# jjhbw/GoMILP

Measured on AMD Instinct MI355X. Metric: simplex pivots/sec on 2048x4096 fp64 dense LP, higher is better.
Workload: dtype f64

## Files before the change

gomilp_amd/csrc/btg_kernels.hip:

```cpp
#include <hip/hip_runtime.h>
#include <hip/hip_ext.h>
#include <stdint.h>

#include <algorithm>
#include <type_traits>

#include "device_types.h"
#include "kernels_common.h"
#include "bt_loop.h"

namespace gomilp {

namespace {

struct XWin { double m; unsigned int i; double p0, p1, p2, p3; };
struct BtWinG { double m; unsigned int i; };

}

template <int G, int NT, int RI, int KR, bool STAMP, bool LOOP = false>
__device__ __forceinline__ void bt_innerG_body(const BTArgs &a, const int g, const int nupd = 0) {
    constexpr int NW = NT / 64;
    static_assert(!LOOP || KR == 16 || KR == 24 || KR == 32, "loop mode: KR / 2 lagging + KR / 2 current terms");
    constexpr int KB = LOOP ? KR / 2 : KR;
    static_assert(G == 2 || G == 4 || G == 8 || G == 16, "G");
#ifdef GOMILP_DEBUG
    if (a.fault && g == 1) return;
#endif
    __shared__ double redM[16];
    __shared__ unsigned int redI[16];
    __shared__ double pay[16][4];
    __shared__ int s_ok;
    __shared__ unsigned long long s_acc[STAMP ? 16 : 1][16];
    unsigned long long tprev = 0;
    auto stamp = [&](int seg) {
        if constexpr (STAMP) {
            unsigned long long t;
            __builtin_amdgcn_sched_barrier(0);
            asm volatile("s_memtime %0\n\ts_waitcnt lgkmcnt(0)" : "=s"(t)::"memory");
            __builtin_amdgcn_sched_barrier(0);
            if (seg >= 0 && (threadIdx.x & 63) == 0) s_acc[threadIdx.x >> 6][seg] += t - tprev;
            tprev = t;
        }
    };
    DevState *st = a.st;
    const int tid = threadIdx.x, lane = tid & 63, wv = tid >> 6;
    const int wbase = __builtin_amdgcn_readfirstlane(tid & ~63);
    const int done = __hip_atomic_load(&st->done, __ATOMIC_RELAXED, __HIP_MEMORY_SCOPE_AGENT);
    long long xs = (long long)a.xbuf[0];
    xpair *recs = reinterpret_cast<xpair *>(a.xbuf + kXHeader);
    const double inf = __builtin_inf();
    const unsigned int ldt = (unsigned int)a.ldt;
    const char *Tb = reinterpret_cast<const char *>(a.T);
    auto ldT = [&](unsigned int elem) -> double {
        if constexpr (LOOP) return ld_agent(reinterpret_cast<const double *>(Tb + (elem << 3)));
// ... 28 lines not shown
    auto hand_on = [&](int nb) {
        hdr_out[0] = (double)(unsigned int)(blk_base + (unsigned int)G * (unsigned int)nb);
#pragma unroll
        for (int j = 0; j < 4; j++) hdr_out[1 + j] = (double)(unsigned int)(upd_base[j] + (unsigned int)nupd * (unsigned int)(nb > j ? (nb - 1 - j) / 4 + 1 : 0));
    };
    if (done) {
        if constexpr (LOOP) {
            if (tid == 0) {
                if (g == 0) {
                    __hip_atomic_store(&st->kdone2[0], 0, __ATOMIC_RELAXED, __HIP_MEMORY_SCOPE_AGENT);
                    asm volatile("s_waitcnt vmcnt(0)" ::: "memory");
                }
                __hip_atomic_fetch_add(blk_cnt, 1u, __ATOMIC_RELAXED, __HIP_MEMORY_SCOPE_AGENT);
                if (g == 0) {
                    st->tsel2[a.par ^ 1] = sel0;
                    st->loop_blocks = 0;
                    hand_on(1);
                }
            }
        } else if (g == 0 && tid == 0) st->kdone = 0;
        return;
    }
    double ureg[RI][KR], vreg[RI][KR];
#pragma unroll
    for (int s = 0; s < RI; s++) {
#pragma unroll
        for (int j = 0; j < KR; j++) { ureg[s][j] = 0; vreg[s][j] = 0; }
    }
    if constexpr (STAMP) { if (tid < 256) s_acc[tid >> 4][tid & 15] = 0; }
    __syncthreads();
    int kd = 0, status = ST_RUNNING, blands = 0;
    bool dead = false;
    long long trace_len = 0, npiv = 0;
    if (g == 0 && tid == 0) { trace_len = st->trace_len; npiv = st->pivots; }

    auto wave_first_min = [&](const double (&val)[RI]) -> BtWinG {
        double x = val[0];
#pragma unroll
        for (int s = 1; s < RI; s++) x = vmin_f64(x, val[s]);
        BtWinG w;
        w.m = wave_min_f64(x);
        w.i = 0xFFFFFFFFu;
#pragma unroll
        for (int s = RI - 1; s >= 0; s--) {
            const unsigned long long mask = __ballot(val[s] == w.m);
            if (mask) w.i = (unsigned int)((s * G + g) * NT + wbase + __builtin_ctzll(mask));
        }
        return w;
    };
    auto xchg = [&](int which) -> XWin {
        stamp(which * 5 + 0);
        if constexpr (!LOOP) asm volatile("s_waitcnt vmcnt(0)" ::: "memory");
        __syncthreads();
        stamp(which * 5 + 1);
        xs += 1;
        const double seqd = (double)xs;
        const int par = (int)(xs & 1);
        if (wv == 0) {
            double fm, v0;
            unsigned int fi;
            if constexpr (LOOP && (NW == 4 || NW == 8)) {
                const double mw = lane < NW ? redM[lane & (NW - 1)] : inf;
                const double iw = lane < NW ? (double)redI[lane & (NW - 1)] : 4294967295.0;
                double xm = mw;
                xm = vmin_f64(xm, dpp_f64<0xB1>(xm));
                xm = vmin_f64(xm, dpp_f64<0x4E>(xm));
// ... 91 lines not shown
            XLoad<1>::run(src, got, fast);
            if (__all(!act || got[0].x == seqd)) break;
            if (++spins > kXSpinLimit) { dead = true; break; }
        }
        stamp(which * 5 + 3);
        const double val = got[0].y;
        double xm = (lane < G) ? val : inf;
        xm = vmin_f64(xm, dpp_f64<0xB1>(xm));
        xm = vmin_f64(xm, dpp_f64<0x4E>(xm));
        xm = vmin_f64(xm, dpp_f64<0x141>(xm));
        const double idxl = dpp_f64<0x108>(val);
        const bool mine = lane < G && val == xm;
        double km = mine ? idxl : 4294967295.0;
        km = vmin_f64(km, dpp_f64<0xB1>(km));
        km = vmin_f64(km, dpp_f64<0x4E>(km));
        km = vmin_f64(km, dpp_f64<0x141>(km));
        const unsigned int mk = (unsigned int)(__ballot(mine && idxl == km) & 0xFFull);
        const int gw = mk ? __builtin_ctz(mk) : 0;
        const double bm = readlane_f64(xm, 0), bi = readlane_f64(km, 0);
        XWin r;
        r.m = bm;
        r.i = (unsigned int)bi;
        r.p0 = readlane_f64(val, 16 + gw);
        r.p1 = readlane_f64(val, 24 + gw);
        r.p2 = readlane_f64(val, 32 + gw);
        r.p3 = readlane_f64(val, 48 + gw);
        if (first) {
            fast = !dead && __all(!(act && (lane >> 3) == 5) || val == (double)myxcc);
            first = false;
        }
        stamp(which * 5 + 4);
        return r;
    };
    auto reduce_cols = [&](const double (&val)[RI]) -> XWin {
        const BtWinG w = wave_first_min(val);
#pragma unroll
        for (int s = 0; s < RI; s++)
            if ((unsigned int)gidx(s) == w.i) {
                pay[wv][0] = rv[s];
                pay[wv][1] = (double)nbasv[s];
                pay[wv][3] = vreg[s][0];
            }
        if (lane == 0) { redM[wv] = w.m; redI[wv] = w.i; }
        return xchg(0);
    };
    auto reduce_rows = [&](const double (&val)[RI], const double (&dcol)[RI]) -> XWin {
        const BtWinG w = wave_first_min(val);
#pragma unroll
        for (int s = 0; s < RI; s++)
            if ((unsigned int)gidx(s) == w.i) {
                pay[wv][0] = dcol[s];
                pay[wv][1] = xbv[s];
                pay[wv][2] = (double)basv[s];
                pay[wv][3] = ureg[s][0];
            }
        if (lane == 0) { redM[wv] = w.m; redI[wv] = w.i; }
        return xchg(1);
    };
    auto column = [&](int q, int k, double (&dcol)[RI], double newest) {
        double d0[RI];
#pragma unroll
        for (int s = 0; s < RI; s++) {
            const int i = gidx(s);
            const unsigned int ic = (unsigned int)(i < a.m ? i : a.m - 1);
            d0[s] = ldT(tile_off_g(ic, (unsigned int)q, ldt));
        }
        double vq[KR];
        if constexpr (LOOP) {
            const int l = lane & 31;
            const int trow = l < k ? cur0 + k - 1 - l : lag0 + nl - 1 - (l - k);
            double tv = l < k + nl ? ld_term(a.V + (size_t)trow * a.ldt + q) : 0.0;
            if (l == 0 && k + nl > 0) tv = newest;
            if constexpr (STAMP) { asm volatile("s_waitcnt vmcnt(0)" ::: "memory"); stamp(11); }
#pragma unroll
            for (int jj = 0; jj < KR; jj++) vq[jj] = readlane_f64(tv, jj);
        } else {
#pragma unroll
            for (int jj = 0; jj < KR; jj++) vq[jj] = jj < k ? ld_term(a.V + (size_t)(k - 1 - jj) * a.ldt + q) : 0.0;
        }
#pragma unroll
// ... 185 lines not shown
            if (j < a.ldt) {
                double v;
                if constexpr (LOOP) {
                    double acc[4] = {0, 0, 0, 0};
#pragma unroll
                    for (int jj = 0; jj < KR; jj++) acc[jj & 3] = __builtin_fma(up[jj], vreg[s][jj], acc[jj & 3]);
                    v = vrow[s] + ((acc[0] + acc[1]) + (acc[2] + acc[3]));
                } else {
                    v = vrow[s];
#pragma unroll
                    for (int jj = 0; jj < KR; jj++) v = __builtin_fma(up[jj], vreg[s][jj], v);
                }
                rv[s] = (j == q) ? -mult : __builtin_fma(-mult, v, rv[s]);
                const double vprime = (j == q) ? dpv + 1.0 : v;
                st_term(Vk + j, vprime);
#pragma unroll
                for (int jj = KR - 1; jj > 0; jj--) vreg[s][jj] = vreg[s][jj - 1];
                vreg[s][0] = vprime;
                if (j == q && commit_lists) nbasv[s] = lea;
            }
        }
        if constexpr (STAMP && !LOOP) asm volatile("s_waitcnt vmcnt(0)" ::: "memory");
        stamp(10);
        if (forced && a.forced_nocommit == 3) status = ST_FORCED_DONE;
        if (g == 0 && tid == 0 && !(forced && a.forced_nocommit)) {
            if (a.trace && trace_len < a.trace_cap) {
                DevPivot &tr = a.trace[trace_len];
                tr.phase = a.phase; tr.bland = bland ? 1 : 0; tr.min_idx = q; tr.replace = p; tr.entering = ent; tr.leaving = lea;
            }
            trace_len += 1;
            npiv += 1;
        }
        kd = k + 1;
    }
    nbe = blk + 1;
    if constexpr (LOOP) {
        if (dead) status = ST_XCHG_TIMEOUT;
        asm volatile("s_waitcnt vmcnt(0)" ::: "memory");
        __syncthreads();
        if (tid == 0) {
            if (g == 0) {
                __hip_atomic_store(&st->kdone2[blk & 1], kd, __ATOMIC_RELAXED, __HIP_MEMORY_SCOPE_AGENT);
                if (status != ST_RUNNING) {
                    __hip_atomic_store(&st->status, status, __ATOMIC_RELAXED, __HIP_MEMORY_SCOPE_AGENT);
                    __hip_atomic_store(&st->done, 1, __ATOMIC_RELAXED, __HIP_MEMORY_SCOPE_AGENT);
                }
                asm volatile("s_waitcnt vmcnt(0)" ::: "memory");
            }
            __hip_atomic_fetch_add(blk_cnt, 1u, __ATOMIC_RELAXED, __HIP_MEMORY_SCOPE_AGENT);
        }
        if (status != ST_RUNNING) break;
    }
    }
    if (dead) status = ST_XCHG_TIMEOUT;
    if constexpr (STAMP) {
        if (a.stamps && g == 0 && lane == 0) {
            for (int sg = 0; sg < 16; sg++) a.stamps[wv * 16 + sg] += s_acc[wv][sg];
            if (wv == 0) a.stamps[16 * 16] += (unsigned long long)kd;
        }
    }
#pragma unroll
    for (int s = 0; s < RI; s++) {
        const int i = gidx(s);
        if (i < a.ldt) a.r[i] = i < a.nn ? rv[s] : 0.0;
        if (i < a.ldu) a.xb[i] = xbv[s];
        if (i < a.m) a.basic[i] = basv[s];
        if (i < a.nn) a.nonbasic[i] = nbasv[s];
    }
    if (tid == 0 && (g == 0 || dead)) {
        if (g == 0) {
            st->trace_len = trace_len;
            st->pivots = npiv;
            if constexpr (LOOP) {
                const int napplied = kd > 0 ? nbe : nbe - 1;
                st->tsel2[a.par ^ 1] = sel0 ^ (napplied & 1);
                st->loop_blocks = nbe;
                hand_on(nbe);
            } else {
                st->kdone = kd;
            }
            st->bland_steps += blands;
            a.xbuf[0] = (double)xs;
        }
        if (status != ST_RUNNING) { st->done = 1; st->status = status; }
    }
}

template <int G, int NT, int RI, int KR, bool STAMP = false>
__global__ __launch_bounds__(NT) void k_bt_innerG(BTArgs a) {
    if (blockIdx.x & 7u) return;
    bt_innerG_body<G, NT, RI, KR, STAMP>(a, (int)(blockIdx.x >> 3));
}
template <int G, int NT, int RI, bool STAMP = false, int KB = 8>
__global__ __launch_bounds__(NT) void k_bt_loop(BTArgs a) {
    const int b = (int)blockIdx.x, x = a.xcd & 7;
    const int nupd = (a.upd_cap > 0 && a.upd_cap < (int)gridDim.x - G) ? a.upd_cap : (int)gridDim.x - G;
    if ((b & 7) == x && (b >> 3) < G) { bt_innerG_body<G, NT, RI, 2 * KB, STAMP, true>(a, b >> 3, nupd); return; }
    const int before = b <= x ? 0 : min(G, ((b - x - 1) >> 3) + 1);
    if (b - before >= nupd) return;
    bt_loop_update_role<NT, KB>(a, b - before, nupd, G);
}

template <int G, int NT, int RI, int KR>
__global__ __launch_bounds__(NT) void k_bt_innerG_batch(const BatchLP *__restrict__ lps, const int *__restrict__ ids, const int *__restrict__ count, int xcd_off) {
    const unsigned int x8 = ((blockIdx.x & 7u) + 8u - (unsigned int)xcd_off) & 7u, j = blockIdx.x >> 3;
    const int lpos = (int)((j / G) * 8u + x8);
    if (lpos >= *count) return;
    const BatchLP &lp = lps[ids[lpos]];
    const int stage = lp.stage;
    if (stage == BS_DONE || stage == BS_HOST) return;
    const BTArgs a = lp.bt;
    bt_innerG_body<G, NT, RI, KR, false>(a, (int)(j % G));
}


size_t bt_xbuf_doubles() { return (size_t)kXSync + kXSyncDoubles; }

BtGroupCfg bt_group_cfg(int m, int ldt, int knob) {
    BtGroupCfg c = {0, 0, 0};
    if (knob < 0) return c;
    const int need = m > ldt ? m : ldt;
    auto fits = [&](int G, int nt, int ri) { return (long)G * nt * ri >= need; };
    if (knob == 16) {
        if (need <= 2048) c = {8, 256, 1};
        else if (need <= 4096) c = {8, 512, 1};
        return c;
    }
    if (knob == 2 || knob == 4 || knob == 8) {
        const int G = knob;
        if (fits(G, 512, 1)) c = {G, 512, 1};
        else if (fits(G, 512, 2)) c = {G, 512, 2};
        return c;
    }
    if (knob != 0) return c;
    if (need <= 1024) return c;
    if (need <= 2048) return {8, 256, 1};
    if (need <= 4096) return {8, 512, 1};
    if (need <= 8192) return {8, 512, 2};
    return c;
}

template <int G, int NT, int RI>
static void btg_launch(const BTArgs &a, hipStream_t s, hipEvent_t e0, hipEvent_t e1) {
    if constexpr (RI == 1) {
        if (a.stamps) { hipExtLaunchKernelGGL((k_bt_innerG<G, NT, RI, 16, true>), dim3(8 * G), dim3(NT), 0, s, e0, e1, 0, a); return; }
    }
    hipExtLaunchKernelGGL((k_bt_innerG<G, NT, RI, 16>), dim3(8 * G), dim3(NT), 0, s, e0, e1, 0, a);
}
void launch_bt_inner_groups(const BTArgs &a, hipStream_t s, hipEvent_t e0, hipEvent_t e1) {
    const int G = a.groups, ri = a.group_ri;
    if (a.group_nt == 256) { btg_launch<8, 256, 1>(a, s, e0, e1); return; }
    if (G == 2) { if (ri == 1) btg_launch<2, 512, 1>(a, s, e0, e1); else btg_launch<2, 512, 2>(a, s, e0, e1); }
    else if (G == 4) { if (ri == 1) btg_launch<4, 512, 1>(a, s, e0, e1); else btg_launch<4, 512, 2>(a, s, e0, e1); }
    else { if (ri == 1) btg_launch<8, 512, 1>(a, s, e0, e1); else btg_launch<8, 512, 2>(a, s, e0, e1); }
}
bool bt_loop_supported(const BtGroupCfg &c) { return c.groups >= 2 && c.ri == 1; }
void launch_bt_loop(const BTArgs &a, int ncu, hipStream_t s, hipEvent_t e0, hipEvent_t e1) {
    const int G = a.groups;
    const unsigned int grid = (unsigned int)std::max(ncu, 8 * G);
    if (a.group_nt == 256 && G == 8) {
        if (a.stamps) hipExtLaunchKernelGGL((k_bt_loop<8, 256, 1, true>), dim3(grid), dim3(256), 0, s, e0, e1, 0, a);
        else hipExtLaunchKernelGGL((k_bt_loop<8, 256, 1>), dim3(grid), dim3(256), 0, s, e0, e1, 0, a);
        return;
    }
    if (G == 16 && a.group_nt == 128) { hipExtLaunchKernelGGL((k_bt_loop<16, 128, 1, false, 8>), dim3(std::max(grid, 136u)), dim3(128), 0, s, e0, e1, 0, a); return; }
    if (G == 16 && a.kmax == 12) { hipExtLaunchKernelGGL((k_bt_loop<16, 256, 1, false, 12>), dim3(std::max(grid, 136u)), dim3(256), 0, s, e0, e1, 0, a); return; }
    if (G == 16) { hipExtLaunchKernelGGL((k_bt_loop<16, 256, 1, false, 16>), dim3(std::max(grid, 128u)), dim3(256), 0, s, e0, e1, 0, a); return; }
    if (G == 2) hipExtLaunchKernelGGL((k_bt_loop<2, 512, 1>), dim3(grid), dim3(512), 0, s, e0, e1, 0, a);
    else if (G == 4) hipExtLaunchKernelGGL((k_bt_loop<4, 512, 1>), dim3(grid), dim3(512), 0, s, e0, e1, 0, a);
    else if (a.kmax == 16) hipExtLaunchKernelGGL((k_bt_loop<8, 512, 1, false, 16>), dim3(grid), dim3(512), 0, s, e0, e1, 0, a);
    else hipExtLaunchKernelGGL((k_bt_loop<8, 512, 1>), dim3(grid), dim3(512), 0, s, e0, e1, 0, a);
}
void launch_bt_inner_groups_batch(const BatchLP *lps, const int *ids, const int *count, int nlp, const BtGroupCfg &c, hipStream_t s, hipEvent_t e0, hipEvent_t e1, int xcd_off) {
    const unsigned int grid = 64u * (unsigned int)((nlp + 7) / 8);
    if (c.nt == 256) hipExtLaunchKernelGGL((k_bt_innerG_batch<8, 256, 1, 16>), dim3(grid), dim3(256), 0, s, e0, e1, 0, lps, ids, count, xcd_off);
    else hipExtLaunchKernelGGL((k_bt_innerG_batch<8, 512, 1, 16>), dim3(grid), dim3(512), 0, s, e0, e1, 0, lps, ids, count, xcd_off);
}
const char *bt_group_kernel_name(int G, int ri) {
    static const char *names[3][2] = {{"k_bt_innerG<2,512,1,16>", "k_bt_innerG<2,512,2,16>"}, {"k_bt_innerG<4,512,1,16>", "k_bt_innerG<4,512,2,16>"},
                                      {"k_bt_innerG<8,512,1,16>", "k_bt_innerG<8,512,2,16>"}};
    return names[G == 2 ? 0 : G == 4 ? 1 : 2][ri == 1 ? 0 : 1];
}

}
```

gomilp_amd/csrc/c_api.cpp:

```cpp
#include <math.h>
#include <stdint.h>
#include <stdio.h>
#include <stdlib.h>
#include <string.h>

#include <atomic>
#include <chrono>
#include <condition_variable>
#include <deque>
#include <functional>
#include <map>
#include <memory>
#include <mutex>
#include <string>
#include <thread>
#include <vector>

#include "engine.hpp"
#include "engine_batch.hpp"
#include "engine_batch_revised.hpp"
#include "lu_host.h"

using gomilp::BatchEngine;
using gomilp::Engine;
// ... 696 lines not shown
    return norm * gomilp::inverse_norm1_estimate(inv, (int)n, inf != 0);
}

int gomilp_debug_gonum_lu_cond(const double *M, int64_t n, int transposed, double *cond) {
    if (!M || !cond || n < 1 || n > gomilp::kGonumCondMax) return -1;
    bool dz = false;
    if (!gomilp::gonum_lu_cond(M, (int)n, (int)n, transposed != 0, cond, &dz)) return -1;
    return dz ? 1 : 0;
}

int gomilp_debug_lu_host_solve(int64_t m, int64_t nd, const int32_t *dl, const int32_t *phys, const double *diag, const double *W, int coupled,
                               const double *rhs, double *x) {
    if (m < 1 || m > 16384 || nd < 0 || nd > m || !phys || !diag || !rhs || !x || (nd > 0 && (!dl || !W))) return -1;
    const int64_t nx = coupled ? nd : m;
    for (int64_t i = 0; i < nx; i++) x[i] = 0.0;
    if (gomilp::lu_det_is_zero(diag, phys, (int)m)) return 1;
    if (coupled) {
        std::vector<double> xdl((size_t)nd);
        gomilp::lu_host_solve_coupled((int)nd, dl, phys, diag, W, rhs, xdl.data(), x);
    } else gomilp::lu_host_solve((int)m, (int)nd, dl, phys, diag, W, rhs, x);
    return 0;
}

int64_t gomilp_debug_find_independent_device(gomilp_ctx *ctx, int64_t problem, int64_t *idx_out, int64_t cap) {
    if (!ctx || !idx_out) return -GOMILP_ERR_BAD_SHAPE;
    std::vector<int32_t> idx;
    const int rc = ctx->eng->debug_find_independent(problem, idx);
    if (rc != GOMILP_OK && rc != GOMILP_ERR_SINGULAR) return -rc;
    for (size_t k = 0; k < idx.size() && (int64_t)k < cap; k++) idx_out[k] = idx[k];
    return (int64_t)idx.size();
}

long long gomilp_debug_loop_rep_launches(void) { return gomilp::bt_loop_rep_launches(); }
#ifdef GOMILP_DEBUG
void gomilp_debug_luc_stamps(unsigned long long *out) { gomilp::luc_stamps_read(out); }
void gomilp_debug_lux_stamps(unsigned long long *out) { gomilp::lux_stamps_read(out); }
void gomilp_debug_res_stamps(unsigned long long *out) { gomilp::res_stamps_read(out); }
#endif

int64_t gomilp_lp_last_trace(gomilp_ctx *ctx, gomilp_pivot *out, int64_t cap) {
    if (!ctx) return -1;
    return ctx->eng->last_trace(out, cap);
}

namespace {
constexpr int kFlatMaxCtx = 32;
struct FlatPool {
    std::mutex mu;
    std::condition_variable cv;
    std::vector<gomilp_ctx *> free_list;
    int created = 0;
};
FlatPool &flat_pool(int dev) {
    static std::mutex mu;
    static std::map<int, FlatPool *> pools;
    std::lock_guard<std::mutex> g(mu);
    auto it = pools.find(dev);
    if (it == pools.end()) it = pools.emplace(dev, new FlatPool).first;
    return *it->second;
}
}

int gomilp_lp_simplex(const double *c, const double *A, int64_t lda, const double *b, int64_t m, int64_t n, double tol,
                      const int64_t *initial_basic, double *opt_f, double *opt_x, int32_t *has_x, int64_t *basis_out,
                      gomilp_lp_stats *stats) {
    if (has_x) *has_x = 0;
// ... 37 lines not shown
```

gomilp_amd/csrc/device_types.h:

```cpp
#pragma once
#include <stdint.h>
#include <stdlib.h>

#ifdef GOMILP_DEBUG
#define GOMILP_DBG_ENV(name) getenv(name)
#else
#define GOMILP_DBG_ENV(name) (static_cast<const char *>(nullptr))
#endif

namespace gomilp {

enum : int32_t {
    ST_RUNNING = 0,
    ST_OPTIMAL = 1,
    ST_UNBOUNDED = 2,
    ST_NEED_BLAND = 3,
    ST_MAX_PIVOTS = 4,
    ST_LU_SINGULAR = 5,
    ST_BLAND_FAILED = 6,
    ST_FORCED_DONE = 7,
    ST_XCHG_TIMEOUT = 9,
    ST_DUAL_INFEASIBLE = 11,
    ST_NEED_EXACT = 10
};
// ... 84 lines not shown
    double *pd_ratio, *px_ratio;
    DevState *st;
    DevPivot *trace;
    int64_t trace_cap;
};

struct BTArgs {
    int32_t m, nn;
    int32_t ldt, ldu;
    int32_t phase, kmax;
    double tol;
    double *T;
    double *U;
    double *V;
    double *r, *xb;
    int32_t *basic, *nonbasic;
    DevState *st;
    DevPivot *trace;
    int64_t trace_cap;
    int32_t forced_q, forced_p, forced_nocommit;
    int32_t nt_force;
    int32_t tiled, old_only;
    unsigned long long *stamps;
    double *xbuf;
    int32_t groups, group_ri;
    int32_t fault, upd_cap;
    int32_t group_nt, upd_valu;
    double *Tbuf[2];
    int32_t loop, nblocks;
    int32_t par, xcd;
    double guard;
    double cguard;
    int32_t exact_once, poll_delay;
};

struct BtGroupCfg { int groups, nt, ri; };

enum : int32_t {
    BS_FORCED = 0,
    BS_P2_START = 1,
    BS_P1 = 2,
    BS_P2 = 3,
    BS_EXCH = 6,
    BS_DONE = 4,
    BS_HOST = 5,
    BS_DUAL_START = 7,
    BS_DUAL = 8,
    BS_COLD = 9
};

struct BatchLP {
    BTArgs bt;
    const double *At0;
    const double *c0, *b0;
    const int32_t *rho0;
    const int32_t *var;
    const double *sign, *rhs;
    int32_t ld0, m0, n0, K;
    int32_t m, n;
    int32_t ldu, cap_ldt;
    double *T[2];
    double *R, *xb, *U, *V, *scratch, *art;
    int32_t *basic, *nonbasic, *srcpos;
    DevState *st;
    const double *gT0;
    const double *gxb0;
// ... 87 lines not shown
```

gomilp_amd/csrc/engine.cpp:

```cpp
#include "engine_work.hpp"

#include <condition_variable>
#include <atomic>

namespace gomilp {

int device_count() {
    int n = 0;
    if (hipGetDeviceCount(&n) != hipSuccess) return 0;
    return n;
}

const char *compiled_arch() { return "gfx950"; }

Engine::Engine(int device) : device_(device), w_(new Work) {}

Engine::~Engine() {
    hipSetDevice(device_);
    if (up_dA_) hipFree(up_dA_);
    if (up_stats_) hipFree(up_stats_);
    for (auto *vec : {&problems_, &child_pool_, &root_pool_})
        for (auto &p : *vec) {
            if (!p) continue;
            hipFree(p->dAt); hipFree(p->db);
// ... 41 lines not shown
    LoopSlots &L = loop_slots(dev);
    {
        std::lock_guard<std::mutex> lk(L.mu);
        if (weight >= 4) { L.used = 0; for (bool &b2 : L.busy) b2 = false; }
        else { L.used--; L.busy[slot & 3] = false; }
    }
    L.cv.notify_all();
}

int Engine::set(const std::string &key, int64_t v) {
    std::lock_guard<std::mutex> g(mu_);
    if (key == "chunk") { if (v < 1) return GOMILP_ERR_BAD_SHAPE; chunk_ = v; }
    else if (key == "refresh") { if (v < 0) return GOMILP_ERR_BAD_SHAPE; refresh_ = v; }
    else if (key == "trace") trace_on_ = v ? 1 : 0;
    else if (key == "max_pivots") max_pivots_ = v < 0 ? 0 : v;
    else if (key == "sample_events") sample_events_ = v < 0 ? 0 : v;
    else if (key == "fused") fused_ = v ? 1 : 0;
    else if (key == "lu_look") lu_look_ = v ? 1 : 0;
    else if (key == "lu_large") lu_large_ = v ? 1 : 0;
    else if (key == "lu_blocked") lu_blocked_ = v < 0 ? 0 : (v > 2 ? 3 : v);
    else if (key == "tableau") tableau_ = v ? 1 : 0;
    else if (key == "blocked") blocked_ = v ? 1 : 0;
    else if (key == "bt_nt") { if (v != 0 && v != 256 && v != 512 && v != 1024) return GOMILP_ERR_BAD_SHAPE; bt_nt_ = v; }
    else if (key == "bt_old") bt_old_ = v ? 1 : 0;
    else if (key == "bt_upd_valu") bt_upd_valu_ = v ? 1 : 0;
#ifdef GOMILP_DEBUG
    else if (key == "bt_fault") bt_fault_ = v;
#endif
    else if (key == "general_device") general_device_ = v ? 1 : 0;
    else if (key == "lu_cross") lu_cross_ = v < 0 ? -1 : (v > 2 ? 2 : v);
    else if (key == "general_block") general_block_ = v ? 1 : 0;
    else if (key == "general_min_rows") general_min_rows_ = v < 2 ? 2 : v;
    else if (key == "bt_groups") { if (v != -1 && v != 0 && v != 2 && v != 4 && v != 8 && v != 16) return GOMILP_ERR_BAD_SHAPE; bt_groups_ = v; }
    else if (key == "bt_stamps") bt_stamps_ = v ? 1 : 0;
    else if (key == "bt_lag") bt_lag_ = v ? 1 : 0;
    else if (key == "exact_degenerate") { if (v < 0 || v > 3) return GOMILP_ERR_BAD_SHAPE; exact_degenerate_ = v; }
    else if (key == "loop_grid") { if (v < 0 || v > 4096) return GOMILP_ERR_BAD_SHAPE; loop_grid_ = v; }
    else if (key == "loop_chunk") { if (v < 32) return GOMILP_ERR_BAD_SHAPE; loop_chunk_ = v; }
    else if (key == "cond_guard") cond_guard_ = v ? 1 : 0;
    else if (key == "poll_delay") { if (v < 0 || v > 64) return GOMILP_ERR_BAD_SHAPE; poll_delay_ = v; }
    else if (key == "loop_upd") { if (v < 0) return GOMILP_ERR_BAD_SHAPE; loop_upd_ = v; }
    else if (key == "loop_rep") loop_rep_ = v ? 1 : 0;
    else if (key == "loop_g") { if (v != 0 && v != 8 && v != 16) return GOMILP_ERR_BAD_SHAPE; loop_g_ = v; }
    else if (key == "loop_k") { if (v != 0 && v != 8 && v != 12 && v != 16) return GOMILP_ERR_BAD_SHAPE; loop_k_ = v; }
    else if (key == "row_chunk") { if (v < 0 || v % 512 != 0 || v > kLdsWindowLd) return GOMILP_ERR_BAD_SHAPE; row_chunk_ = v; }
    else if (key == "block_k") { if (v < 0 || v > bt_max_k()) return GOMILP_ERR_BAD_SHAPE; block_k_ = v; }
    else return GOMILP_ERR_BAD_SHAPE;
    return GOMILP_OK;
}

int Engine::ensure_work(int m, int ncols) {
    HIP_TRY(hipSetDevice(device_));
    if (!stream_) HIP_TRY(hipStreamCreateWithFlags(&stream_, hipStreamNonBlocking));
    Work &w = *w_;
    if (!w.st) {
        int ncu = 0;
        if (hipDeviceGetAttribute(&ncu, hipDeviceAttributeMultiprocessorCount, device_) == hipSuccess && ncu > 0) ncu_ = ncu;
        HIP_TRY(dmalloc(&w.pk_price, 2 * kMaxPartials)); HIP_TRY(dmalloc(&w.pk_ratio, 2 * kMaxPartials));
        HIP_TRY(dmalloc(&w.pi_price, kMaxPartials)); HIP_TRY(dmalloc(&w.pi_ratio, kMaxPartials));
        HIP_TRY(dmalloc(&w.pv_price, kMaxPartials)); HIP_TRY(dmalloc(&w.pb_ratio, kMaxPartials)); HIP_TRY(dmalloc(&w.pd_ratio, kMaxPartials)); HIP_TRY(dmalloc(&w.px_ratio, kMaxPartials));
        for (int t = 0; t < 2; t++) {
            HIP_TRY(dmalloc(&w.lpk[t], kMaxPartials)); HIP_TRY(dmalloc(&w.lpl[t], kMaxPartials)); HIP_TRY(dmalloc(&w.lpr[t], kMaxPartials));
        }
        HIP_TRY(dmalloc(&w.st, 1));
        HIP_TRY(hipHostMalloc(reinterpret_cast<void **>(&w.st_host), sizeof(DevState), hipHostMallocDefault));
        HIP_TRY(dmalloc(&w.luctl, 2));
        HIP_TRY(hipHostMalloc(reinterpret_cast<void **>(&w.luctl_host), 2 * sizeof(LUCtl), hipHostMallocDefault));
// ... 1311 lines not shown
```

gomilp_amd/csrc/engine.hpp:

```cpp
#pragma once
#include <hip/hip_runtime_api.h>
#include <stdint.h>

#include <functional>
#include <map>
#include <memory>
#include <mutex>
#include <string>
#include <vector>

#include "../../include/gomilp_lp.h"
#include "device_types.h"

namespace gomilp {

constexpr int kLdsWindowLd = 8192;
constexpr int kAutoRowChunk = 4096;

struct Problem {
    int m = 0, n = 0, ld = 0;
    double *dAt = nullptr;
    double *dc = nullptr;
    double *dc1 = nullptr;
    double *db = nullptr;
// ... 160 lines not shown
    int cond_check(const Problem &P, int nn, double *k1, double *kinf);
    int cond_fresh(const Problem &P, const int32_t *basic_host, double *k1, double *kinf);
    int groups_knob(const Problem &P) const;
    bool ensure_host_A(const Problem &P);
    int find_independent_device(const Problem &P, std::vector<int32_t> &basic, std::vector<double> *binv_out, bool *binv_on_device = nullptr);
    int stage_upload(void *dst, const void *src, size_t bytes);
    hipError_t sync_stream();
    int upload_index_lists(const std::vector<int32_t> &basic, const std::vector<int32_t> &nonbasic);
    void sync_state_to_device();

    int device_;
    hipStream_t stream_ = nullptr;
    int ncu_ = 256;
    std::mutex mu_;
    std::vector<std::unique_ptr<Problem>> problems_;
    std::vector<std::unique_ptr<Problem>> child_pool_;
    std::vector<std::unique_ptr<Problem>> root_pool_;
    double *up_dA_ = nullptr; size_t up_dA_cap_ = 0;
    int32_t *up_stats_ = nullptr; size_t up_stats_cap_ = 0;
    std::unique_ptr<Work> w_;
    int64_t lu_look_faults_ = 0;
    int lu_look_fault_ = 0;
    int64_t lu_look_ = 1;
    int64_t lu_large_ = 0;
    int64_t chunk_ = 32, refresh_ = 0, trace_on_ = 0, max_pivots_ = 0, sample_events_ = 0, fused_ = 1, lu_blocked_ = 3, tableau_ = 1, blocked_ = 1, block_k_ = 0,
            bt_nt_ = 0, bt_old_ = 0, bt_stamps_ = 0, bt_upd_valu_ = 0, bt_fault_ = 0, general_device_ = 1, general_block_ = 1, general_min_rows_ = 96, lu_cross_ = -1, bt_groups_ = 0,
            bt_lag_ = 1,
            loop_chunk_ = 512,
            loop_grid_ = 0,
            poll_delay_ = 0,
            loop_upd_ = 0,
            loop_rep_ = 0,
            loop_g_ = 0,
            loop_k_ = 0,
            exact_degenerate_ = 1,
            cond_guard_ = 1,
            row_chunk_ = 0;
    bool lds_window_only_ = false;
    bool badly_scaled_ = false;
    bool gen_binv_dev_ = false;
    bool gen_start_ = false;
    bool gen_revised_ = false;
    double lp_guard_ = 0.0;
    std::vector<double> exact_xb_;
    bool xchg_timeout_ = false;
    bool shadow_trace_ = false;
    int cur_ = 0;
    int ycur_ = 0;
    int grid_ratio_ = 1;
    int tcur_ = 0, rcur_ = 0, ldt_ = 0;
    bool t_tiled_ = false;
    bool use_bt_ = false;
    int64_t launches_ = 0;
    double fs_device_ = 0, fs_host_ = 0;
    int64_t lu_dense_ = 0, lu_rounds_ = 0;
    std::vector<gomilp_pivot> last_trace_;
    int64_t last_trace_total_ = 0;
};

int general_find_linearly_independent(const std::vector<double> &A, int m, int n, std::vector<int32_t> &idxs, std::vector<double> *binv_out = nullptr);
int general_finish_last_column(const std::vector<double> &A, int m, int n, std::vector<int32_t> &idxs, int start_col, std::vector<double> *binv_out);
int general_find_linearly_independent_slow(const std::vector<double> &A, int m, int n, std::vector<int32_t> &idxs);
bool general_basis_inverse(const std::vector<double> &A, int m, int n, const std::vector<int32_t> &basic, int ncols_with_art,
                           const std::vector<double> &art, std::vector<double> &binv);

int general_condition_replay(const std::vector<double> &A, int m, int n, std::vector<int32_t> &basic, const std::vector<std::pair<int, int>> &pivots,
// ... 41 lines not shown
void launch_gs_init(double *QT, int ldq, int m, GsState *st, hipStream_t s);
void launch_gs_init_perm(double *QT, double *Rinv, int ldq, int m, const int32_t *perm, const double *sgn, const double *beta, int s0, GsState *st, hipStream_t s);
void launch_gs_candidate(const double *acol, double *QT, double *Rinv, int ldq, int m, double *w, double *t, double *ypart, int cand, int32_t *idxs, GsState *st, hipStream_t s,
                         int last = 0);
int launch_luc_rounds_cross(const LUArgs &base, int32_t *pivrow, int nrounds, int round_base, double *xrec, int G, int slots, hipStream_t s);
size_t luc_cross_doubles();
void launch_luc_lpos_final(const LUArgs &a, hipStream_t s);
int luc_cross_groups(int m, int want);
int luc_large_rpt(int m);
int gs_scratch_rows();
int gs_block_width(int m);
int gs_block_scratch_rows();
void launch_gs_block(const double *At, int ld, int col0, int ncand, double *QT, double *Rinv, int ldq, int m, double *scratch, int32_t *idxs, GsState *st, hipStream_t s);
void launch_gs_binv(const double *Rinv, const double *QT, int ldq, int m, double *C, hipStream_t s);
void launch_gs_art(const double *At, int ld, int m, const int32_t *basic, int minidx, const double *b, double *art, hipStream_t s);
void launch_gs_norms(const double *C, int ldq, int m, double *out, const double *At, int ld, const int32_t *idxs, int cand, double *colsum, hipStream_t s);
bool bt_supported(int m, int nn);
int bt_max_k();
int bt_reg_k(int m, int ldt, int nt_force);
bool bt_tiled(int m, int ldt, int kmax, int nt_force, bool old_only);
BtGroupCfg bt_group_cfg(int m, int ldt, int knob);
size_t bt_xbuf_doubles();
void launch_bt_inner_groups(const BTArgs &a, hipStream_t s, hipEvent_t e0, hipEvent_t e1);
const char *bt_group_kernel_name(int G, int ri);
constexpr int kBtStampSegs = 16;
void launch_bt_tile(const double *src, double *dst, int m, int ldt, bool to_tiles, hipStream_t s);
void launch_bt_inner(const BTArgs &a, hipStream_t s, hipEvent_t e0, hipEvent_t e1);
void launch_bt_update(const BTArgs &a, hipStream_t s, hipEvent_t e0, hipEvent_t e1);
bool bt_loop_supported(const BtGroupCfg &c);
void launch_bt_loop(const BTArgs &a, int ncu, hipStream_t s, hipEvent_t e0, hipEvent_t e1);
bool bt_loop_rep_supported(int m, int ldt);
int bt_loop_rep_threads(int m, int ldt);
long long bt_loop_rep_launches();
void launch_bt_loop_rep(const BTArgs &a, int ncu, hipStream_t s, hipEvent_t e0, hipEvent_t e1);
bool bt_batch_supported(int m_max, int ldt_max);
int bt_batch_k(int m_max, int ldt_max);
void launch_bt_inner_batch(const BatchLP *lps, const int *ids, const int *count, int nlp, int m_max, int ldt_max, hipStream_t s, hipEvent_t e0 = nullptr, hipEvent_t e1 = nullptr, int xcd_off = 0);
void launch_bt_update_batch(const BatchLP *lps, const int *ids, const int *count, int nlp, int m_max, int ldt_max, hipStream_t s, hipEvent_t e0 = nullptr, hipEvent_t e1 = nullptr);
const char *bt_batch_kernel_name(int m_max, int ldt_max);
bool bt_virt_batch_supported(int m_max, int ldt_max);
void launch_bt_inner_virt_batch(const BatchLP *lps, const int *ids, const int *count, int nlp, hipStream_t s, hipEvent_t e0 = nullptr, hipEvent_t e1 = nullptr);
int b_loop_slots(int ncu);
bool b_loop_supported(int m_max, int ldt_max);
void launch_b_loop(const BatchLP *lps, const int *ids, const int *count, int nlp, int nblocks, int par, hipStream_t s, hipEvent_t e0 = nullptr, hipEvent_t e1 = nullptr);
size_t b_res_slot_bytes();
int b_res_max_slots();
int b_res_groups(int m_max, int nn_max, int ldt_max);
void launch_b_res(const BatchLP *lps, const int *ids, const int *count, int nlp, int G, int nb, double seq0, void *xbase, hipStream_t s, hipEvent_t e0 = nullptr, hipEvent_t e1 = nullptr);
int batch_ldt(int nn);
void launch_b_setup(BatchLP *lps, int nlp, hipStream_t s);
void launch_b_setup_warm(BatchLP *lps, int nlp, hipStream_t s);
void launch_b_posvar(const int32_t *basic, int m, const int32_t *nonbasic, int nn, int32_t *posvar, hipStream_t s);
bool bt_dual_batch_supported(int m_max, int ldt_max);
void launch_bt_inner_dual_batch(const BatchLP *lps, const int *ids, const int *count, int nlp, int m_max, int ldt_max, hipStream_t s);
void launch_b_gather(const BatchLP *lps, int nlp, int m_max, int ldt_max, int mode, hipStream_t s);
void launch_b_write_virt(const BatchLP *lps, const int *ids, const int *count, int *list, int *nalive, int bound, int m_max, int ldt_max, int ncu, hipStream_t s);
void launch_b_ctrl(BatchLP *lps, const int *ids_in, const int *count_in, int bound, int n_max, BatchOut *outs, int *ids_out, int *count_out, int loop_par, hipStream_t s);
void launch_b_init_ids(int *ids, int *count, int nlp, hipStream_t s);
void launch_b_permute(const BatchLP *lps, const int *ids, const int *count, int bound, int m_max, int ldt_max, hipStream_t s);
void launch_b_tab_r(const BatchLP *lps, const int *ids, const int *count, int bound, int m_max, int ldt_max, hipStream_t s);
void launch_transpose_in(const double *A, int64_t lda, int m, int n, double *At, int ld, hipStream_t s);
void launch_col_stats(const double *At, int ld, int m, int n, int32_t *nnz, int32_t *lastrow, int32_t *allone, int32_t *rowflag, unsigned long long *range,
                      hipStream_t s);
void launch_set_binv_perm(double *binv, int ld, int m, const int32_t *rho, hipStream_t s);
void launch_child_assemble(const double *At0, int ld0, int m0, int n0, double *At1, int ld1, int K, const int32_t *var,
                           const double *sign, hipStream_t s);
// ... 24 lines not shown
```

gomilp_amd/csrc/engine_tableau.cpp:

```cpp
#include <stdio.h>
#include <stdlib.h>

#include "engine_work.hpp"

namespace gomilp {

TabArgs Engine::make_tab_args(const Problem &P, int phase, double tol, int nn) {
    Work &w = *w_;
    TabArgs a;
    memset(&a, 0, sizeof(a));
    a.m = P.m; a.nn = nn; a.ldt = ldt_; a.phase = phase; a.tol = tol;
    bt_layout(P, false);
    a.T_cur = w.T[tcur_]; a.T_next = w.T[tcur_ ^ 1];
    a.r_in = w.R[rcur_]; a.r_out = w.R[rcur_ ^ 1];
    a.xb = w.xb; a.dvec = w.dvec; a.move = w.move;
    a.basic = w.basic; a.nonbasic = w.nonbasic;
    a.pk_ratio = w.pk_ratio; a.pi_ratio = w.pi_ratio; a.pb_ratio = w.pb_ratio; a.pd_ratio = w.pd_ratio; a.px_ratio = w.px_ratio;
    a.st = w.st;
    a.trace = (trace_on_ || shadow_trace_) ? w.trace : nullptr;
    a.trace_cap = w.trace_cap;
    return a;
}

int Engine::tab_forced_pivot(const Problem &P, int phase, double tol, int nn, int q, int ent, double rq, int p, double dp,
// ... 350 lines not shown
        if ((rc = lu_solve(P, dsol, col.data())) != GOMILP_OK) return -rc;
        bool neg = false;
        for (int t = 0; t < m; t++) {
            double d = -dsol[t];
            if (fabs(d) < 1e-13) d = 0;
            if (d < 0) neg = true;
            move[t] = d >= 0 ? std::numeric_limits<double>::infinity() : xb[t] / fabs(d);
        }
        if (!neg) return 2;
        const int64_t rp0 = min_idx(move.data(), m);
        if (fabs(move[rp0]) > 1e-12) { *q_out = i; *p_out = (int)rp0; return 0; }
        for (int rp = 0; rp < m; rp++) {
            if (move[rp] > 1e-12) continue;
            std::vector<int32_t> trial = basic;
            trial[rp] = var;
            const double kappa = general_basis_cond1(P.hA, m, n, trial, art);
            if (kappa < 1e16) { *q_out = i; *p_out = rp; return 0; }
        }
    }
    return -GOMILP_ERR_BLAND;
}

int Engine::run_loop_bt(const Problem &P, int phase, double tol, int nn, gomilp_lp_stats *st) {
    Work &w = *w_;
    DevState &hs = *w.st_host;
    hs.done = 0; hs.status = ST_RUNNING; hs.pivots = 0; hs.kdone = 0; hs.bland_steps = 0; hs.lu_singular = 0;
    int K; bool tiled_plan, lag;
    bt_plan(P, &K, &tiled_plan, &lag);
    struct LoopSlot {
        int dev, weight, slot = -1;
        LoopSlot(int d, int w2, bool on) : dev(d), weight(w2) { if (on) slot = Engine::loop_acquire(d, w2); }
        ~LoopSlot() { if (slot >= 0) Engine::loop_release(dev, weight, slot); }
    };
    const bool small_loop = lag && (K == 8 || K == 16) && loop_g_ != 8 && !bt_stamps_ && bt_group_cfg(P.m, ldt_, groups_knob(P)).nt == 256;
    const BtGroupCfg gc0 = bt_group_cfg(P.m, ldt_, groups_knob(P));
    const bool rep_ok = lag && K == 8 && loop_rep_ && loop_g_ != 8 && gc0.groups == 8 && gc0.nt == 256 && gc0.ri == 1 && bt_loop_rep_supported(P.m, ldt_);
    struct RepHold {
        int dev; bool held;
        RepHold(int d, bool want) : dev(d), held(want && Engine::loop_try_acquire_all(d)) {}
        ~RepHold() { if (held) Engine::loop_release(dev, 4, 0); }
    } rep_hold(device_, rep_ok);
    LoopSlot loop_slot(device_, small_loop ? 1 : 4, lag && !rep_hold.held);
    const int loop_xcd = (small_loop && loop_slot.slot > 0) ? 2 * loop_slot.slot : 0;
    bt_layout(P, tiled_plan);
    hs.tsel2[0] = hs.tsel2[1] = tcur_; hs.kdone2[0] = hs.kdone2[1] = 0; hs.loop_blocks = 0;
    sync_state_to_device();
    if (bt_stamps_) {
        const size_t nb = (size_t)(16 * kBtStampSegs + 8) * sizeof(unsigned long long);
        if (!w.stamps) {
            HIP_TRY(hipMalloc(reinterpret_cast<void **>(&w.stamps), nb));
            HIP_TRY(hipHostMalloc(reinterpret_cast<void **>(&w.stamps_host), nb, hipHostMallocDefault));
        }
        HIP_TRY(hipMemsetAsync(w.stamps, 0, nb, stream_));
    }
    const double t_loop0 = now_s();
    int ret = GOMILP_OK;
    const int64_t blocks_per_chunk = lag ? std::max<int64_t>(4, loop_chunk_ / K) : std::max<int64_t>(1, chunk_ / K);
    const bool sampling = sample_events_ > 0;
    int64_t block_no = 0;
    int64_t &launch_no = w.loop_launches;
    if (!w.pipe_state[0]) {
        for (int t = 0; t < 2; t++) {
            HIP_TRY(hipHostMalloc(reinterpret_cast<void **>(&w.pipe_state[t]), sizeof(DevState), hipHostMallocDefault));
            HIP_TRY(hipEventCreateWithFlags(&w.pipe_ev[t], hipEventDisableTiming));
        }
    }
    struct ChunkInfo { int64_t before_pred; size_t samp0, nsamp; int64_t nblocks; int par; };
    int last_slot_enqueued = 0;
    bool exact_pending = false;
    int forced_q_pending = -1, forced_p_pending = -1;
    int64_t seg0 = 0;
    ChunkInfo info[2];
    size_t samp_total = 0;
    auto enqueue_chunk = [&](int slot, int64_t before_pred, int64_t nblocks) -> int {
        info[slot].before_pred = before_pred;
        info[slot].samp0 = samp_total;
        info[slot].nsamp = 0;
        info[slot].nblocks = nblocks;
        info[slot].par = (int)(launch_no & 1);
        last_slot_enqueued = slot;
        if (lag) {
            BTArgs ai = make_bt_args(P, phase, tol, nn, K);
            ai.loop = 1; ai.nblocks = (int)nblocks; ai.par = (int)(launch_no & 1);
            if (ai.groups == 8 && ai.group_nt == 512 && ai.group_ri == 1 && loop_g_ != 8 && (K == 16 || K == 12)) { ai.groups = 16; ai.group_nt = 256; }
            const bool k16_small = ai.groups == 8 && ai.group_nt == 256 && ai.group_ri == 1 && loop_g_ != 8 && K == 16;
            if (k16_small) ai.groups = 16;
            const bool rep = rep_hold.held && ai.groups == 8 && ai.group_nt == 256 && ai.group_ri == 1;
            if (rep) { ai.groups = 16; ai.group_nt = bt_loop_rep_threads(P.m, ldt_); }
            else if (ai.groups == 8 && ai.group_nt == 256 && ai.group_ri == 1 && loop_g_ != 8 && K == 8 && !bt_stamps_) {
                ai.groups = 16; ai.group_nt = 128;
            }
            ai.Tbuf[0] = w.T[0]; ai.Tbuf[1] = w.T[1];
            ai.xcd = loop_xcd; ai.upd_cap = (int)loop_upd_; ai.poll_delay = (int)poll_delay_;
            if (ai.upd_cap == 0 && ai.groups == 16 && ai.group_nt == 256 && !k16_small) ai.upd_cap = 112;
            ai.exact_once = exact_pending ? 1 : 0; exact_pending = false;
            ai.forced_q = forced_q_pending; ai.forced_p = forced_p_pending; forced_q_pending = forced_p_pending = -1;
            hipEvent_t e0 = nullptr, e1 = nullptr;
            if (sampling) {
                while (w.sample_ev.size() < (samp_total + 1) * 6) { hipEvent_t ev; HIP_TRY(hipEventCreate(&ev)); w.sample_ev.push_back(ev); }
                e0 = w.sample_ev[samp_total * 6]; e1 = w.sample_ev[samp_total * 6 + 1];
                samp_total++; info[slot].nsamp++;
            }
            int grid = (int)std::min<int64_t>(ncu_, std::max<int64_t>(64, (int64_t)P.m * ldt_ * 8 / (256 << 10)));
            if (loop_grid_ > 0) grid = (int)loop_grid_;
            if (rep) launch_bt_loop_rep(ai, grid, stream_, e0, e1);
            else launch_bt_loop(ai, grid, stream_, e0, e1);
            launch_no++; block_no += nblocks; launches_++;
            HIP_TRY(hipMemcpyAsync(w.pipe_state[slot], w.st, sizeof(DevState), hipMemcpyDeviceToHost, stream_));
            HIP_TRY(hipEventRecord(w.pipe_ev[slot], stream_));
            return GOMILP_OK;
        }
        for (int64_t bkk = 0; bkk < nblocks; bkk++, block_no++) {
            int kmax = K;
            if (max_pivots_ > 0) kmax = (int)std::max<int64_t>(1, std::min<int64_t>(K, max_pivots_ - before_pred - bkk * K));
            BTArgs a = make_bt_args(P, phase, tol, nn, kmax);
            a.kmax = K;
            BTArgs ai = a; ai.kmax = kmax;
            ai.exact_once = exact_pending ? 1 : 0; exact_pending = false;
            ai.forced_q = forced_q_pending; ai.forced_p = forced_p_pending; forced_q_pending = forced_p_pending = -1;
            const bool sample = sampling && (block_no % std::max<int64_t>(1, sample_events_ / K) == 0);
            hipEvent_t e[4] = {nullptr, nullptr, nullptr, nullptr};
            if (sample) {
                while (w.sample_ev.size() < (samp_total + 1) * 6) { hipEvent_t ev; HIP_TRY(hipEventCreate(&ev)); w.sample_ev.push_back(ev); }
// ... 375 lines not shown
```

Baseline: 212,800.

## Publish per-wave exchange records in G16x128 loop kernel instead of workgroup reduction

Adds a wave-record exchange path for the 16-group, 128-thread persistent loop kernel. Each wave writes its own argmin and payload record directly to the cross-workgroup exchange buffer and all 32 records are polled and reduced in-wave, skipping the intra-workgroup shared-memory reduction and barrier. The path is enabled by default through a new knob. In exchange, twice as many records must be polled per exchange, the record layout is denser, and a tie-break path is added for equal minima.

```diff
diff --git a/gomilp_amd/csrc/btg_kernels.hip b/gomilp_amd/csrc/btg_kernels.hip
--- a/gomilp_amd/csrc/btg_kernels.hip
+++ b/gomilp_amd/csrc/btg_kernels.hip
@@ -3,6 +3,7 @@
 #include <stdint.h>
 
 #include <algorithm>
+#include <atomic>
 #include <type_traits>
 
 #include "device_types.h"
@@ -18,9 +19,10 @@
 
 }
 
-template <int G, int NT, int RI, int KR, bool STAMP, bool LOOP = false>
+template <int G, int NT, int RI, int KR, bool STAMP, bool LOOP = false, bool WREC = false>
 __device__ __forceinline__ void bt_innerG_body(const BTArgs &a, const int g, const int nupd = 0) {
     constexpr int NW = NT / 64;
+    static_assert(!WREC || (LOOP && G == 16 && NW == 2 && RI == 1), "wave records: two half-line records per workgroup, 32 in all");
     static_assert(!LOOP || KR == 16 || KR == 24 || KR == 32, "loop mode: KR / 2 lagging + KR / 2 current terms");
     constexpr int KB = LOOP ? KR / 2 : KR;
     static_assert(G == 2 || G == 4 || G == 8 || G == 16, "G");
@@ -115,6 +117,7 @@
     int kd = 0, status = ST_RUNNING, blands = 0;
     bool dead = false;
     long long trace_len = 0, npiv = 0;
+    unsigned long long spiv = 0;
     if (g == 0 && tid == 0) { trace_len = st->trace_len; npiv = st->pivots; }
 
     auto wave_first_min = [&](const double (&val)[RI]) -> BtWinG {
@@ -272,8 +275,77 @@
         stamp(which * 5 + 4);
         return r;
     };
+    auto xchg_wave = [&](int which, const BtWinG w, double v1, int id1, double v2, double v3) -> XWin {
+        typedef unsigned long long xtag2 __attribute__((ext_vector_type(2)));
+        stamp(which * 5 + 0);
+        stamp(which * 5 + 1);
+        xs += 1;
+        const unsigned int seq32 = (unsigned int)xs;
+        const int par = (int)(xs & 1);
+        const int wl = w.i != 0xFFFFFFFFu ? (int)(w.i & 63u) : 0;
+        const unsigned long long b1 = (unsigned long long)__double_as_longlong(readlane_f64(v1, wl));
+        const unsigned int i1 = (unsigned int)__builtin_amdgcn_readlane(id1, wl);
+        const unsigned long long b2 = (unsigned long long)__double_as_longlong(readlane_f64(v2, wl));
+        const unsigned long long b3 = (unsigned long long)__double_as_longlong(readlane_f64(v3, wl));
+        if (lane < 4) {
+            const unsigned int ti = (lane == 0 ? w.i : 0u) | (lane == 1 ? i1 : 0u) | (lane == 2 ? myxcc : 0u);
+            xtag2 v;
+            v.x = ((unsigned long long)seq32 << 32) | ti;
+            v.y = (lane == 0 ? (unsigned long long)__double_as_longlong(w.m) : 0ull) | (lane == 1 ? b1 : 0ull) | (lane == 2 ? b2 : 0ull) | (lane == 3 ? b3 : 0ull);
+            xstore(recs + ((size_t)(par * G + g) * kXSlots + 4 * wv + lane), __builtin_bit_cast(xpair, v), fast);
+        }
+        stamp(which * 5 + 2);
+        for (int dl = 0; dl < a.poll_delay; dl++) __builtin_amdgcn_s_sleep(1);
+        const int h = lane & 31;
+        const xpair *src = recs + (size_t)par * G * kXSlots + (h >> 1) * kXSlots + (h & 1) * 4 + 2 * (lane >> 5);
+        xpair got[2];
+        xtag2 t0, t1;
+        int spins = 0;
+        for (;;) {
+            XLoad<2>::run(src, src + 1, got, fast);
+            t0 = __builtin_bit_cast(xtag2, got[0]);
+            t1 = __builtin_bit_cast(xtag2, got[1]);
+            if (__all((unsigned int)(t0.x >> 32) == seq32 && (unsigned int)(t1.x >> 32) == seq32)) break;
+            if (++spins > kXSpinLimit) { dead = true; break; }
+        }
+        stamp(which * 5 + 3);
+        const double val = got[0].y, val2 = got[1].y;
+        const unsigned int idx = (unsigned int)t0.x, id = (unsigned int)t1.x;
+        double xm = lane < 32 ? val : inf;
+        xm = vmin_f64(xm, dpp_f64<0xB1>(xm));
+        xm = vmin_f64(xm, dpp_f64<0x4E>(xm));
+        xm = vmin_f64(xm, dpp_f64<0x141>(xm));
+        xm = vmin_f64(xm, dpp_f64<0x140>(xm));
+        xm = vmin_f64(xm, bcast_f64<0x142, 0xA>(xm));
+        const double bm = readlane_f64(xm, 31);
+        const bool mine = lane < 32 && val == bm;
+        const unsigned int mk0 = (unsigned int)__ballot(mine);
+        int hw;
+        if (__builtin_popcount(mk0) == 1) hw = __builtin_ctz(mk0);
+        else {
+            const unsigned int ki = row_min_u32(mine ? idx : 0xFFFFFFFFu);
+            const unsigned int kmin = min((unsigned int)__builtin_amdgcn_readlane((int)ki, 0), (unsigned int)__builtin_amdgcn_readlane((int)ki, 16));
+            const unsigned int mk = (unsigned int)__ballot(mine && idx == kmin);
+            hw = mk ? __builtin_ctz(mk) : 0;
+        }
+        XWin r;
+        r.m = bm;
+        r.i = (unsigned int)__builtin_amdgcn_readlane((int)idx, hw);
+        r.p0 = readlane_f64(val2, hw);
+        const double wid = (double)__builtin_amdgcn_readlane((int)id, hw);
+        r.p1 = which == 0 ? wid : readlane_f64(val, 32 + hw);
+        r.p2 = wid;
+        r.p3 = readlane_f64(val2, 32 + hw);
+        if (first) {
+            fast = !dead && __all(lane < 32 || idx == myxcc);
+            first = false;
+        }
+        stamp(which * 5 + 4);
+        return r;
+    };
     auto reduce_cols = [&](const double (&val)[RI]) -> XWin {
         const BtWinG w = wave_first_min(val);
+        if constexpr (WREC) return xchg_wave(0, w, rv[0], nbasv[0], 0.0, vreg[0][0]);
 #pragma unroll
         for (int s = 0; s < RI; s++)
             if ((unsigned int)gidx(s) == w.i) {
@@ -286,6 +358,7 @@
     };
     auto reduce_rows = [&](const double (&val)[RI], const double (&dcol)[RI]) -> XWin {
         const BtWinG w = wave_first_min(val);
+        if constexpr (WREC) return xchg_wave(1, w, dcol[0], basv[0], xbv[0], ureg[0][0]);
 #pragma unroll
         for (int s = 0; s < RI; s++)
             if ((unsigned int)gidx(s) == w.i) {
@@ -537,6 +610,7 @@
             npiv += 1;
         }
         kd = k + 1;
+        if constexpr (STAMP) spiv += 1;
     }
     nbe = blk + 1;
     if constexpr (LOOP) {
@@ -561,7 +635,7 @@
     if constexpr (STAMP) {
         if (a.stamps && g == 0 && lane == 0) {
             for (int sg = 0; sg < 16; sg++) a.stamps[wv * 16 + sg] += s_acc[wv][sg];
-            if (wv == 0) a.stamps[16 * 16] += (unsigned long long)kd;
+            if (wv == 0) a.stamps[16 * 16] += LOOP ? spiv : (unsigned long long)kd;
         }
     }
 #pragma unroll
@@ -596,11 +670,11 @@
     if (blockIdx.x & 7u) return;
     bt_innerG_body<G, NT, RI, KR, STAMP>(a, (int)(blockIdx.x >> 3));
 }
-template <int G, int NT, int RI, bool STAMP = false, int KB = 8>
+template <int G, int NT, int RI, bool STAMP = false, int KB = 8, bool WREC = false>
 __global__ __launch_bounds__(NT) void k_bt_loop(BTArgs a) {
     const int b = (int)blockIdx.x, x = a.xcd & 7;
     const int nupd = (a.upd_cap > 0 && a.upd_cap < (int)gridDim.x - G) ? a.upd_cap : (int)gridDim.x - G;
-    if ((b & 7) == x && (b >> 3) < G) { bt_innerG_body<G, NT, RI, 2 * KB, STAMP, true>(a, b >> 3, nupd); return; }
+    if ((b & 7) == x && (b >> 3) < G) { bt_innerG_body<G, NT, RI, 2 * KB, STAMP, true, WREC>(a, b >> 3, nupd); return; }
     const int before = b <= x ? 0 : min(G, ((b - x - 1) >> 3) + 1);
     if (b - before >= nupd) return;
     bt_loop_update_role<NT, KB>(a, b - before, nupd, G);
@@ -660,6 +734,8 @@
     else { if (ri == 1) btg_launch<8, 512, 1>(a, s, e0, e1); else btg_launch<8, 512, 2>(a, s, e0, e1); }
 }
 bool bt_loop_supported(const BtGroupCfg &c) { return c.groups >= 2 && c.ri == 1; }
+static std::atomic<long long> g_wave_rec_launches{0};
+long long bt_loop_wave_rec_launches() { return g_wave_rec_launches.load(); }
 void launch_bt_loop(const BTArgs &a, int ncu, hipStream_t s, hipEvent_t e0, hipEvent_t e1) {
     const int G = a.groups;
     const unsigned int grid = (unsigned int)std::max(ncu, 8 * G);
@@ -668,7 +744,16 @@
         else hipExtLaunchKernelGGL((k_bt_loop<8, 256, 1>), dim3(grid), dim3(256), 0, s, e0, e1, 0, a);
         return;
     }
-    if (G == 16 && a.group_nt == 128) { hipExtLaunchKernelGGL((k_bt_loop<16, 128, 1, false, 8>), dim3(std::max(grid, 136u)), dim3(128), 0, s, e0, e1, 0, a); return; }
+    if (G == 16 && a.group_nt == 128) {
+        const dim3 g16(std::max(grid, 136u));
+        if (a.wave_rec) g_wave_rec_launches++;
+        if (a.stamps) {
+            if (a.wave_rec) hipExtLaunchKernelGGL((k_bt_loop<16, 128, 1, true, 8, true>), g16, dim3(128), 0, s, e0, e1, 0, a);
+            else hipExtLaunchKernelGGL((k_bt_loop<16, 128, 1, true, 8, false>), g16, dim3(128), 0, s, e0, e1, 0, a);
+        } else if (a.wave_rec) hipExtLaunchKernelGGL((k_bt_loop<16, 128, 1, false, 8, true>), g16, dim3(128), 0, s, e0, e1, 0, a);
+        else hipExtLaunchKernelGGL((k_bt_loop<16, 128, 1, false, 8, false>), g16, dim3(128), 0, s, e0, e1, 0, a);
+        return;
+    }
     if (G == 16 && a.kmax == 12) { hipExtLaunchKernelGGL((k_bt_loop<16, 256, 1, false, 12>), dim3(std::max(grid, 136u)), dim3(256), 0, s, e0, e1, 0, a); return; }
     if (G == 16) { hipExtLaunchKernelGGL((k_bt_loop<16, 256, 1, false, 16>), dim3(std::max(grid, 128u)), dim3(256), 0, s, e0, e1, 0, a); return; }
     if (G == 2) hipExtLaunchKernelGGL((k_bt_loop<2, 512, 1>), dim3(grid), dim3(512), 0, s, e0, e1, 0, a);
diff --git a/gomilp_amd/csrc/c_api.cpp b/gomilp_amd/csrc/c_api.cpp
--- a/gomilp_amd/csrc/c_api.cpp
+++ b/gomilp_amd/csrc/c_api.cpp
@@ -752,6 +752,7 @@
 }
 
 long long gomilp_debug_loop_rep_launches(void) { return gomilp::bt_loop_rep_launches(); }
+long long gomilp_debug_loop_wave_rec_launches(void) { return gomilp::bt_loop_wave_rec_launches(); }
 #ifdef GOMILP_DEBUG
 void gomilp_debug_luc_stamps(unsigned long long *out) { gomilp::luc_stamps_read(out); }
 void gomilp_debug_lux_stamps(unsigned long long *out) { gomilp::lux_stamps_read(out); }
diff --git a/gomilp_amd/csrc/device_types.h b/gomilp_amd/csrc/device_types.h
--- a/gomilp_amd/csrc/device_types.h
+++ b/gomilp_amd/csrc/device_types.h
@@ -140,6 +140,7 @@
     double guard;
     double cguard;
     int32_t exact_once, poll_delay;
+    int32_t wave_rec, pad_;
 };
 
 struct BtGroupCfg { int groups, nt, ri; };
diff --git a/gomilp_amd/csrc/engine.cpp b/gomilp_amd/csrc/engine.cpp
--- a/gomilp_amd/csrc/engine.cpp
+++ b/gomilp_amd/csrc/engine.cpp
@@ -97,7 +97,8 @@
     else if (key == "general_block") general_block_ = v ? 1 : 0;
     else if (key == "general_min_rows") general_min_rows_ = v < 2 ? 2 : v;
     else if (key == "bt_groups") { if (v != -1 && v != 0 && v != 2 && v != 4 && v != 8 && v != 16) return GOMILP_ERR_BAD_SHAPE; bt_groups_ = v; }
-    else if (key == "bt_stamps") bt_stamps_ = v ? 1 : 0;
+    else if (key == "bt_stamps") bt_stamps_ = v < 0 ? 0 : (v > 2 ? 2 : v);
+    else if (key == "loop_wave_rec") loop_wave_rec_ = v ? 1 : 0;
     else if (key == "bt_lag") bt_lag_ = v ? 1 : 0;
     else if (key == "exact_degenerate") { if (v < 0 || v > 3) return GOMILP_ERR_BAD_SHAPE; exact_degenerate_ = v; }
     else if (key == "loop_grid") { if (v < 0 || v > 4096) return GOMILP_ERR_BAD_SHAPE; loop_grid_ = v; }
diff --git a/gomilp_amd/csrc/engine.hpp b/gomilp_amd/csrc/engine.hpp
--- a/gomilp_amd/csrc/engine.hpp
+++ b/gomilp_amd/csrc/engine.hpp
@@ -216,6 +216,7 @@
             loop_upd_ = 0,
             loop_rep_ = 0,
             loop_g_ = 0,
+            loop_wave_rec_ = 1,
             loop_k_ = 0,
             exact_degenerate_ = 1,
             cond_guard_ = 1,
@@ -323,6 +324,7 @@
 bool bt_loop_rep_supported(int m, int ldt);
 int bt_loop_rep_threads(int m, int ldt);
 long long bt_loop_rep_launches();
+long long bt_loop_wave_rec_launches();
 void launch_bt_loop_rep(const BTArgs &a, int ncu, hipStream_t s, hipEvent_t e0, hipEvent_t e1);
 bool bt_batch_supported(int m_max, int ldt_max);
 int bt_batch_k(int m_max, int ldt_max);
diff --git a/gomilp_amd/csrc/engine_tableau.cpp b/gomilp_amd/csrc/engine_tableau.cpp
--- a/gomilp_amd/csrc/engine_tableau.cpp
+++ b/gomilp_amd/csrc/engine_tableau.cpp
@@ -406,7 +406,7 @@
         LoopSlot(int d, int w2, bool on) : dev(d), weight(w2) { if (on) slot = Engine::loop_acquire(d, w2); }
         ~LoopSlot() { if (slot >= 0) Engine::loop_release(dev, weight, slot); }
     };
-    const bool small_loop = lag && (K == 8 || K == 16) && loop_g_ != 8 && !bt_stamps_ && bt_group_cfg(P.m, ldt_, groups_knob(P)).nt == 256;
+    const bool small_loop = lag && (K == 8 || K == 16) && loop_g_ != 8 && bt_stamps_ != 1 && bt_group_cfg(P.m, ldt_, groups_knob(P)).nt == 256;
     const BtGroupCfg gc0 = bt_group_cfg(P.m, ldt_, groups_knob(P));
     const bool rep_ok = lag && K == 8 && loop_rep_ && loop_g_ != 8 && gc0.groups == 8 && gc0.nt == 256 && gc0.ri == 1 && bt_loop_rep_supported(P.m, ldt_);
     struct RepHold {
@@ -461,8 +461,8 @@
             if (k16_small) ai.groups = 16;
             const bool rep = rep_hold.held && ai.groups == 8 && ai.group_nt == 256 && ai.group_ri == 1;
             if (rep) { ai.groups = 16; ai.group_nt = bt_loop_rep_threads(P.m, ldt_); }
-            else if (ai.groups == 8 && ai.group_nt == 256 && ai.group_ri == 1 && loop_g_ != 8 && K == 8 && !bt_stamps_) {
-                ai.groups = 16; ai.group_nt = 128;
+            else if (ai.groups == 8 && ai.group_nt == 256 && ai.group_ri == 1 && loop_g_ != 8 && K == 8 && bt_stamps_ != 1) {
+                ai.groups = 16; ai.group_nt = 128; ai.wave_rec = loop_wave_rec_ ? 1 : 0;
             }
             ai.Tbuf[0] = w.T[0]; ai.Tbuf[1] = w.T[1];
             ai.xcd = loop_xcd; ai.upd_cap = (int)loop_upd_; ai.poll_delay = (int)poll_delay_;
```

Measured after the change: 233,600 (median of 6 runs). 1.1x the previous value.
